# ace19-dev/gvcnn-tf

Hardware: NVIDIA B200
Metric: grouping+fusion shapes/s (12-view, D=2048) (higher is better)
Workload: dtype f32

## Files before the change

gvcnn-tf_b200/build.py:

```python
from __future__ import annotations

import os
import shutil
import subprocess
import sys

HERE = os.path.dirname(os.path.abspath(__file__))
ROOT = os.path.dirname(HERE)
CSRC = os.path.join(HERE, "csrc")
SO = os.path.join(HERE, "libgvcnn_sm100.so")
SOURCES = ["capi.cu", "host_pipeline.cu", "comm.cu", "score.cu", "gap_score.cu", "scheme.cu", "pool_fwd.cu", "pool_fwd_ring.cu", "pool_fwd_direct.cu", "pool_gap_ring.cu", "pool_bwd.cu", "pool_bwd_fast.cu", "paper_mode.cu"]
HEADERS = [os.path.join(CSRC, "common.cuh"), os.path.join(CSRC, "ring_common.cuh"), os.path.join(ROOT, "include", "gvcnn_b200.h")]


def nvcc_path():
    for cand in (shutil.which("nvcc"), "/usr/local/cuda/bin/nvcc"):
        if cand and os.path.exists(cand):
            return cand
    raise RuntimeError("nvcc not found: libgvcnn_sm100.so cannot be built (there is no fallback path)")


def needs_build():
    if not os.path.exists(SO):
        return True
    t = os.path.getmtime(SO)
    deps = [os.path.join(CSRC, s) for s in SOURCES] + HEADERS + [os.path.abspath(__file__)]
    return any(os.path.getmtime(d) > t for d in deps)


def build(force=False, verbose=False, defines=(), out=None):
    if out is None and not force and not needs_build():
        return SO
    import concurrent.futures
    import hashlib
    import tempfile
    target = out or SO
    common = [nvcc_path()]
    if os.path.exists("/usr/bin/g++"):
        common += ["-ccbin", "/usr/bin/g++"]
    common += ["-std=c++17", "-O3", "-lineinfo",
               "-gencode", "arch=compute_100a,code=sm_100a",
               "-fmad=false",
               "-Xcompiler", "-fPIC",
               "-I", os.path.join(ROOT, "include"), "-I", CSRC] + ["-D" + d for d in defines]
    if verbose:
        common.insert(1, "-Xptxas=-v")
    tag = hashlib.sha1((" ".join(defines) + target).encode()).hexdigest()[:10]
    objdir = os.path.join(tempfile.gettempdir(), "gvcnn_build_" + tag)
    os.makedirs(objdir, exist_ok=True)

    def compile_one(src):
        obj = os.path.join(objdir, src.replace(".cu", ".o"))
        res = subprocess.run(common + ["-c", os.path.join(CSRC, src), "-o", obj], capture_output=True, text=True)
        return src, obj, res

    log = []
    objs = []
    with concurrent.futures.ThreadPoolExecutor(max_workers=min(len(SOURCES), os.cpu_count() or 4)) as ex:
        for src, obj, res in ex.map(compile_one, SOURCES):
            log.append(res.stdout + res.stderr)
            if res.returncode != 0:
                sys.stderr.write("".join(log))
                raise RuntimeError("nvcc failed compiling %s" % src)
            objs.append(obj)
    link = common[:1] + (["-ccbin", "/usr/bin/g++"] if os.path.exists("/usr/bin/g++") else []) + \
# ... 16 lines not shown
```

gvcnn-tf_b200/csrc/capi.cu:

```cuda
#include <cstdlib>

#include "comm_dev.cuh"

#ifndef GVCNN_FWD_DIRECT
#define GVCNN_FWD_DIRECT 1
#endif

using namespace gvcnn;

namespace {

size_t elt_size(int dtype) { return dtype == GVCNN_F32 ? 4 : 2; }

int make_view_ptrs(const void *X, int layout, int dtype, int B, int V, int64_t D, ViewPtrs &vp, int64_t &sb,
                   bool &aligned16)
{
    if (!X) return GVCNN_E_BAD_ARG;
    const size_t es = elt_size(dtype);
    char *base = const_cast<char *>(static_cast<const char *>(X));
    switch (layout) {
    case GVCNN_LAYOUT_BVD:
        for (int v = 0; v < V; ++v) vp.p[v] = base + (size_t)v * D * es;
        sb = (int64_t)V * D;
        break;
// ... 291 lines not shown
    if (rc) return rc;
    al = al && is_aligned(dS, 16) && (D * es) % 16 == 0 && (!tie_mask || is_aligned(tie_mask, 8));
    if (weights && (!is_aligned(weights, 4) || weight_stride_b < 0)) return GVCNN_E_BAD_ARG;
    if (al && (variant == 0 || variant == 3 || variant == 4)) {
        rc = launch_pool_fuse_bwd_fast(dS, bins, bin_stride_b, tie_mask, weights, weight_stride_b, gp, sb, status, B, V, D, G, pool, dtype,
                                       static_cast<cudaStream_t>(stream));
        if (rc != -1000) return rc;
    }
    return launch_pool_fuse_bwd(dS, bins, bin_stride_b, tie_mask, weights, weight_stride_b, gp, sb, status, B, V, D, G, pool, dtype, al,
                                static_cast<cudaStream_t>(stream));
}

int gvcnn_grouping_fusion_fwd(const void *R, const float *W, const float *bias, const void *F, float *x,
                              float *scores, int32_t *bins, int32_t *flags, void *S, uint8_t *tie_mask,
                              int32_t *status, int B, int V, int C, int64_t D, int G, int pool, float empty_fill,
                              int r_layout, int f_layout, int dtype, int edge_ulps, int clamp, void *stream)
{
    int rc = check_dims(B, V, D, G, dtype);
    if (rc) return rc == kEmptyBatch ? 0 : rc;
    if (C <= 0 || !W || !bias || !scores || !bins || !S || edge_ulps < 0) return GVCNN_E_BAD_ARG;
    if ((pool & 0xff) != GVCNN_POOL_MAX && (pool & 0xff) != GVCNN_POOL_MEAN) return GVCNN_E_BAD_MODE;
    const size_t es = elt_size(dtype);
    ViewPtrs rp, fp;
    int64_t rsb, fsb;
    bool ral, fal;
    rc = make_view_ptrs(R, r_layout, dtype, B, V, C, rp, rsb, ral);
    if (rc) return rc;
    rc = make_view_ptrs(F, f_layout, dtype, B, V, D, fp, fsb, fal);
    if (rc) return rc;
    (void)es;
    rc = gvcnn_score_bin_fwd(R, W, bias, x, scores, bins, flags, status, B, V, C, G, r_layout, dtype, edge_ulps, clamp,
                             stream);
    if (rc) return rc;
    return pool_fuse_fwd_impl(F, bins, V, nullptr, 0, S, nullptr, tie_mask, status, B, V, D, G, pool, empty_fill,
                               f_layout, dtype, true, stream);
}

int gvcnn_grouping_fusion_batch_fwd(const void *R, const float *W, const float *bias, const void *F, float *x,
                                    float *xsum, float *x_mean, float *scores, int32_t *bins, int32_t *flags, void *S,
                                    uint8_t *tie_mask, int32_t *status, int B, int V, int C, int64_t D, int G,
                                    int multiplier, int pool, float empty_fill, int r_layout, int f_layout, int dtype,
                                    int edge_ulps, int clamp, int64_t global_count, gvcnn_exchange_fn exchange,
                                    void *exchange_user, void *stream)
{
    int rc = check_dims(B, V, D, G, dtype);
    if (rc && rc != kEmptyBatch) return rc;
    const bool empty = rc == kEmptyBatch;
    if (empty && !exchange) return 0;
    if (C <= 0 || !W || !bias || !xsum || !scores || !bins || edge_ulps < 0 || multiplier < 0) return GVCNN_E_BAD_ARG;
    if (!empty && (!x || !S)) return GVCNN_E_BAD_ARG;
    if (global_count < B || global_count <= 0) return GVCNN_E_BAD_ARG;
    if ((pool & 0xff) != GVCNN_POOL_MAX && (pool & 0xff) != GVCNN_POOL_MEAN) return GVCNN_E_BAD_MODE;
    cudaStream_t st = static_cast<cudaStream_t>(stream);
    if (!empty) {
        rc = gvcnn_view_score_fwd(R, W, bias, x, nullptr, B, V, C, r_layout, dtype, stream);
        if (rc) return rc;
    }
    rc = batch_score_tail(empty ? nullptr : x, xsum, x_mean, scores, bins, flags, status, B, V, G, multiplier, edge_ulps,
                          clamp, global_count, exchange, exchange_user, st);
    if (rc || empty) return rc;
    return pool_fuse_fwd_impl(F, bins, 0, nullptr, 0, S, nullptr, tie_mask, status, B, V, D, G, pool, empty_fill,
                               f_layout, dtype, true, stream);
}

size_t gvcnn_pool_fuse_gap_workspace_bytes(int B, int C, int HW, int dtype)
{
    if (B <= 0 || C <= 0 || HW <= 0) return 0;
    return gap_workspace_bytes(B, C, HW, dtype);
}

int gvcnn_pool_fuse_gap_fwd(const void *F, const int32_t *bins, int64_t bin_stride_b, void *S_gap, uint8_t *tie_mask,
                            int32_t *status, void *workspace, size_t workspace_bytes, int B, int V, int HW, int C,
                            int G, int pool, float empty_fill, int f_layout, int dtype, void *stream)
{
    if (HW <= 0 || C <= 0) return GVCNN_E_BAD_ARG;
    const int64_t D = (int64_t)HW * C;
    int rc = check_dims(B, V, D, G, dtype);
    if (rc) return rc == kEmptyBatch ? 0 : rc;
    if (!bins || !S_gap || !workspace || bin_stride_b < 0) return GVCNN_E_BAD_ARG;
    if (pool != GVCNN_POOL_MAX && pool != GVCNN_POOL_MEAN) return GVCNN_E_BAD_MODE;
    ViewPtrs fp;
    int64_t sb;
    bool al;
    rc = make_view_ptrs(F, f_layout, dtype, B, V, D, fp, sb, al);
    if (rc) return rc;
    const size_t need = gap_workspace_bytes(B, C, HW, dtype);
    if (!al || need == 0 || V > 32 || (tie_mask && !is_aligned(tie_mask, 8)) || !is_aligned(workspace, 16))
        return GVCNN_E_UNSUPPORTED;
    if (workspace_bytes < need) return GVCNN_E_WORKSPACE;
    rc = launch_pool_fuse_gap_fwd(fp, sb, bins, bin_stride_b, S_gap, tie_mask, status, static_cast<float *>(workspace),
                                  B, V, HW, C, G, pool, empty_fill, dtype, static_cast<cudaStream_t>(stream));
    return rc == -1000 ? GVCNN_E_UNSUPPORTED : rc;
}

int gvcnn_pool_fuse_gap_bwd(const void *dS_gap, const int32_t *bins, int64_t bin_stride_b, const uint8_t *tie_mask,
                            void *dF, int32_t *status, int B, int V, int HW, int C, int G, int pool, int g_layout,
                            int dtype, void *stream)
{
    if (HW <= 0 || C <= 0) return GVCNN_E_BAD_ARG;
    const int64_t D = (int64_t)HW * C;
    int rc = check_dims(B, V, D, G, dtype);
    if (rc) return rc == kEmptyBatch ? 0 : rc;
    if (!dS_gap || !bins || bin_stride_b < 0) return GVCNN_E_BAD_ARG;
    if (pool != GVCNN_POOL_MAX && pool != GVCNN_POOL_MEAN) return GVCNN_E_BAD_MODE;
    if (pool == GVCNN_POOL_MAX && !tie_mask) return GVCNN_E_BAD_ARG;
    ViewPtrs gp;
// ... 72 lines not shown
```

gvcnn-tf_b200/csrc/common.cuh:

```cuda
#pragma once

#include <cuda_bf16.h>
#include <cuda_runtime.h>
#include <stdint.h>

#include <atomic>
#include <cstdlib>

#include "gvcnn_b200.h"

namespace gvcnn {

struct ViewPtrs {
    char *p[GVCNN_MAX_VIEWS];
};

struct Plan {
    int32_t rawbin[GVCNN_MAX_VIEWS];
    int32_t gbin[GVCNN_MAX_VIEWS];
    float gw[GVCNN_MAX_VIEWS];
    float sumw;
    uint16_t glen[GVCNN_MAX_VIEWS];
    uint8_t order[GVCNN_MAX_VIEWS];
};
// ... 418 lines not shown
    const float lo = fmaxf(ax - dx, 0.0f), hi = ax + dx;
    float s_lo = __fdiv_rn(lo, __fadd_rn(1.0f, lo)), s_hi = __fdiv_rn(hi, __fadd_rn(1.0f, hi));
    const uint32_t bl = __float_as_uint(s_lo), bh = __float_as_uint(s_hi);
    s_lo = __uint_as_float(bl > (uint32_t)edge_ulps ? bl - edge_ulps : 0u);
    s_hi = __uint_as_float(bh + edge_ulps);
    const float fg = (float)(mult > 0 ? mult : G);
    return ((int)__fmul_rn(s_lo, fg) != (int)__fmul_rn(s_hi, fg)) ? GVCNN_FLAG_ORDER_EDGE : 0;
}

__device__ __forceinline__ void publish(int flags, int32_t *flag_out, int32_t *status)
{
    if (flag_out) *flag_out = flags;
    if (status && flags) {
        if (flags & GVCNN_FLAG_BIN_RANGE) atomicAdd(status + GVCNN_STATUS_BIN_RANGE, 1);
        if (flags & GVCNN_FLAG_NAN) atomicAdd(status + GVCNN_STATUS_NAN, 1);
        if (flags & GVCNN_FLAG_NEAR_EDGE) atomicAdd(status + GVCNN_STATUS_NEAR_EDGE, 1);
    }
}

int launch_view_score(const ViewPtrs &rp, int64_t r_sb, const float *W, const float *bias, float *x, float *xabs,
                      float *scores, int32_t *bins, int32_t *flags, int32_t *status, int B, int V, int C,
                      int G, int dtype, bool aligned16, bool fuse_bin, int edge_ulps, int clamp,
                      cudaStream_t st);
int launch_gap_score(const ViewPtrs &mp, int64_t m_sb, const float *W, const float *bias, float *R_out, float *x,
                     float *scores, int32_t *bins, int32_t *flags, int32_t *status, int B, int V, int HW, int C, int G,
                     int dtype, bool fuse_bin, int edge_ulps, int clamp, cudaStream_t st);
int launch_batch_sum_x(const float *x, float *xsum, int B, int V, cudaStream_t st);
int launch_score_bin(const float *x, float denom, float *x_mean, float *scores, int32_t *bins, int32_t *flags,
                     int32_t *status, int64_t n, int G, int multiplier, int edge_ulps, int clamp, bool x_is_score,
                     const float *xabs, int bound_terms, cudaStream_t st);
int launch_bins_to_scheme(const int32_t *bins, int32_t *scheme, int rows, int V, int G, cudaStream_t st);
int launch_scheme_to_bins(const int32_t *scheme, int32_t *bins, int32_t *status, int rows, int V, int G,
                          cudaStream_t st);
int launch_group_weight(const int32_t *bins, float *weights, int rows, int V, int G, cudaStream_t st);
int launch_pool_fuse_fwd(const ViewPtrs &fp, int64_t f_sb, const int32_t *bins, int64_t bin_sb, void *S,
                         void *Pout, uint8_t *mask, const float *weights, int64_t w_sb, int32_t *status, int B, int V, int64_t D, int G, int pool,
                         float fill, int dtype, bool aligned16, int variant, cudaStream_t st);
int launch_group_weight_from_scores(const float *scores, const int32_t *bins, float *weights, int rows, int V, int G,
                                    cudaStream_t st);
int launch_group_weight_grad(const ViewPtrs &fp, int64_t f_sb, const void *dS, const void *S, const int32_t *bins,
                             int64_t bin_sb, const float *weights, int64_t w_sb, float *dweights, int B, int V,
                             int64_t D, int G, int pool, int dtype, bool aligned16, cudaStream_t st);
int launch_score_weight_bwd(const float *dweights, const int32_t *bins, const float *x, float *dx, int rows, int V,
                            int G, cudaStream_t st);
int launch_view_score_bwd(const ViewPtrs &rp, int64_t r_sb, const float *dx, const float *W, float *dW, float *dbias,
                          const ViewPtrs &drp, int64_t dr_sb, int want_dr, float *workspace, int NS, int B, int V,
                          int C, int dtype, bool aligned16, cudaStream_t st);
int launch_pool_fuse_fwd_ring(const ViewPtrs &fp, int64_t f_sb, const int32_t *bins, int64_t bin_sb,
                              const float *weights, int64_t w_sb, void *S, uint8_t *mask, int32_t *status, int B, int V, int64_t D, int G, int pool,
                              float fill, int dtype, cudaStream_t st);
int launch_pool_fuse_fwd_direct(const ViewPtrs &fp, int64_t f_sb, const int32_t *bins, int64_t bin_sb, void *S,
                                uint8_t *mask, int32_t *status, int B, int V, int64_t D, int G, int pool, float fill,
                                int dtype, bool forced, bool f_ready, cudaStream_t st);
size_t gap_workspace_bytes(int B, int C, int HW, int dtype);
int launch_pool_fuse_gap_fwd(const ViewPtrs &fp, int64_t f_sb, const int32_t *bins, int64_t bin_sb, void *out,
                             uint8_t *mask, int32_t *status, float *partial, int B, int V, int HW, int C, int G,
                             int pool, float fill, int dtype, cudaStream_t st);
int launch_pool_fuse_gap_bwd(const void *dOut, const int32_t *bins, int64_t bin_sb, const uint8_t *mask,
                             const ViewPtrs &gp, int64_t g_sb, int32_t *status, int B, int V, int HW, int C, int G,
                             int pool, int dtype, cudaStream_t st);
int launch_pool_fuse_bwd_fast(const void *dS, const int32_t *bins, int64_t bin_sb, const uint8_t *mask,
                              const float *weights, int64_t w_sb, const ViewPtrs &gp, int64_t g_sb, int32_t *status, int B, int V, int64_t D, int G,
                              int pool, int dtype, cudaStream_t st);
int launch_pool_fuse_bwd(const void *dS, const int32_t *bins, int64_t bin_sb, const uint8_t *mask,
                         const float *weights, int64_t w_sb,
                         const ViewPtrs &gp, int64_t g_sb, int32_t *status, int B, int V, int64_t D, int G,
                         int pool, int dtype, bool aligned16, cudaStream_t st);

}
```

gvcnn-tf_b200/csrc/score.cu:

```cuda
#include "comm_dev.cuh"

namespace gvcnn {

constexpr int kScoreWarps = 8;
constexpr int kScoreUnroll = 8;

template <typename T, bool VEC, bool FUSE_BIN, bool BOUND>
__global__ void __launch_bounds__(kScoreWarps * 32)
view_score_kernel(const ViewPtrs rp, const int64_t r_sb, const float *__restrict__ W,
                  const float *__restrict__ bias, float *__restrict__ x_out, float *__restrict__ xabs_out,
                  float *__restrict__ scores,
                  int32_t *__restrict__ bins, int32_t *__restrict__ flag_out, int32_t *status, const int B,
                  const int V, const int C, const int G, const int edge_ulps, const int clamp)
{
    constexpr int E = VEC ? Elem<T>::kVec : 1;
    const int lane = threadIdx.x & 31;
    const int64_t row = (int64_t)blockIdx.x * kScoreWarps + (threadIdx.x >> 5);
    pdl_wait();
    pdl_launch_dependents();
    if (row >= (int64_t)B * V) return;
    const int b = (int)(row / V);
    const int v = (int)(row - (int64_t)b * V);
    const T *__restrict__ r = reinterpret_cast<const T *>(rp.p[v]) + (int64_t)b * r_sb;
    const float *__restrict__ w = W + (int64_t)v * C;

    float acc = 0.0f, aabs = 0.0f;
    if constexpr (VEC) {
        for (int base0 = lane * E; base0 < C; base0 += 32 * E * kScoreUnroll) {
            uint4 raw[kScoreUnroll];
#pragma unroll
            for (int u = 0; u < kScoreUnroll; ++u) {
                const int base = base0 + u * 32 * E;
                if (base < C) raw[u] = ldg_stream_16(r + base);
            }
#pragma unroll
            for (int u = 0; u < kScoreUnroll; ++u) {
                const int base = base0 + u * 32 * E;
                if (base < C) {
                    float f[E];
                    Elem<T>::unpack(raw[u], f);
#pragma unroll
                    for (int j = 0; j < E; j += 4) {
                        const float4 wv = __ldg(reinterpret_cast<const float4 *>(w + base + j));
                        acc = fmaf(f[j + 0], wv.x, acc);
                        acc = fmaf(f[j + 1], wv.y, acc);
                        acc = fmaf(f[j + 2], wv.z, acc);
                        acc = fmaf(f[j + 3], wv.w, acc);
                        if constexpr (BOUND) {
                            aabs = fmaf(fabsf(f[j + 0]), fabsf(wv.x), aabs);
                            aabs = fmaf(fabsf(f[j + 1]), fabsf(wv.y), aabs);
                            aabs = fmaf(fabsf(f[j + 2]), fabsf(wv.z), aabs);
                            aabs = fmaf(fabsf(f[j + 3]), fabsf(wv.w), aabs);
                        }
                    }
                }
            }
        }
    } else {
        for (int c = lane; c < C; c += 32) {
            const float rv = Elem<T>::to_float(r[c]), wv = __ldg(w + c);
            acc = fmaf(rv, wv, acc);
            if constexpr (BOUND) aabs = fmaf(fabsf(rv), fabsf(wv), aabs);
        }
    }
#pragma unroll
    for (int off = 16; off >= 1; off >>= 1) acc = __fadd_rn(acc, __shfl_xor_sync(0xffffffffu, acc, off));
    if constexpr (BOUND) {
#pragma unroll
        for (int off = 16; off >= 1; off >>= 1) aabs = __fadd_rn(aabs, __shfl_xor_sync(0xffffffffu, aabs, off));
    }

    if (lane == 0) {
        const float bv = __ldg(bias + v);
        const float x = __fadd_rn(acc, bv);
        const float A = BOUND ? __fadd_rn(aabs, fabsf(bv)) : 0.0f;
        if (x_out) x_out[row] = x;
        if constexpr (BOUND && !FUSE_BIN) xabs_out[row] = A;
        if constexpr (FUSE_BIN) {
            float s;
            int bin;
            int flags = score_and_bin(x, 1.0f, G, edge_ulps, clamp, s, bin);
            if constexpr (BOUND) flags |= order_edge_flag(x, A, C + 2, G, 0, edge_ulps);
            scores[row] = s;
            bins[row] = bin;
            publish(flags, flag_out ? flag_out + row : nullptr, status);
        }
    }
}

constexpr int kFastRows = 4;

__device__ __forceinline__ float transpose_reduce4(const float (&acc)[4], const int lane)
{
    const bool hi = (lane & 16) != 0;
    float k0 = hi ? acc[2] : acc[0], k1 = hi ? acc[3] : acc[1];
    const float s0 = hi ? acc[0] : acc[2], s1 = hi ? acc[1] : acc[3];
    k0 = __fadd_rn(k0, __shfl_xor_sync(0xffffffffu, s0, 16));
    k1 = __fadd_rn(k1, __shfl_xor_sync(0xffffffffu, s1, 16));
    const bool h8 = (lane & 8) != 0;
    float k = h8 ? k1 : k0;
    const float sd = h8 ? k0 : k1;
    k = __fadd_rn(k, __shfl_xor_sync(0xffffffffu, sd, 8));
#pragma unroll
    for (int off = 4; off >= 1; off >>= 1) k = __fadd_rn(k, __shfl_xor_sync(0xffffffffu, k, off));
    return k;
}

template <typename T, int NB, bool BOUND>
__global__ void __launch_bounds__(kScoreWarps * 32)
view_score_fast_kernel(const ViewPtrs rp, const int64_t r_sb, const float *__restrict__ W,
                       const float *__restrict__ bias, float *__restrict__ x_out, float *__restrict__ xabs_out,
                       float *__restrict__ scores,
                       int32_t *__restrict__ bins, int32_t *__restrict__ flag_out, int32_t *status, const int B,
                       const int V, const int G, const int edge_ulps, const int clamp, const int64_t items,
                       const int rpw)
{
    constexpr int E = Elem<T>::kVec;
    constexpr int C = NB * 32 * E;
    const int lane = threadIdx.x & 31;
    const int64_t item = (int64_t)blockIdx.x * kScoreWarps + (threadIdx.x >> 5);
    pdl_wait();
    pdl_launch_dependents();
    if (item >= items) return;
    const int v = (int)(item % V);
    const int b_first = (int)(item / V) * rpw;
    const int b_end = min(b_first + rpw, B);
    const T *__restrict__ r0 = reinterpret_cast<const T *>(rp.p[v]) + lane * E;
    const float *__restrict__ w = W + (int64_t)v * C + lane * E;
    const float bv = __ldg(bias + v);
#ifndef GVCNN_SCORE_PD_MAX
#define GVCNN_SCORE_PD_MAX kFastRows
#endif
    constexpr int PD = (16 / NB) < GVCNN_SCORE_PD_MAX ? (16 / NB < 2 ? 2 : 16 / NB) : GVCNN_SCORE_PD_MAX;
    uint4 buf[PD][NB];
#pragma unroll
    for (int j = 0; j < PD; ++j) {
        if (b_first + j < b_end) {
            const T *rn = r0 + (int64_t)(b_first + j) * r_sb;
#pragma unroll
            for (int u = 0; u < NB; ++u) buf[j][u] = ldg_stream_16(rn + u * 32 * E);
        } else {
#pragma unroll
            for (int u = 0; u < NB; ++u) buf[j][u] = make_uint4(0u, 0u, 0u, 0u);
        }
    }
    for (int b0 = b_first; b0 < b_end; b0 += kFastRows) {
        float acc[kFastRows], aabs[kFastRows];
#pragma unroll
        for (int j = 0; j < kFastRows; ++j) {
            float a = 0.0f, aa = 0.0f;
#pragma unroll
            for (int u = 0; u < NB; ++u) {
                float f[E];
                Elem<T>::unpack(buf[j % PD][u], f);
#pragma unroll
                for (int q = 0; q < E; q += 4) {
                    const float4 wv = __ldg(reinterpret_cast<const float4 *>(w + u * 32 * E + q));
                    a = fmaf(f[q + 0], wv.x, a);
                    a = fmaf(f[q + 1], wv.y, a);
                    a = fmaf(f[q + 2], wv.z, a);
                    a = fmaf(f[q + 3], wv.w, a);
                    if constexpr (BOUND) {
                        aa = fmaf(fabsf(f[q + 0]), fabsf(wv.x), aa);
                        aa = fmaf(fabsf(f[q + 1]), fabsf(wv.y), aa);
                        aa = fmaf(fabsf(f[q + 2]), fabsf(wv.z), aa);
                        aa = fmaf(fabsf(f[q + 3]), fabsf(wv.w), aa);
                    }
                }
            }
            acc[j] = a;
            aabs[j] = aa;
            const int bn = b0 + j + PD;
            if (bn < b_end) {
                const T *rn = r0 + (int64_t)bn * r_sb;
#pragma unroll
                for (int u = 0; u < NB; ++u) buf[j % PD][u] = ldg_stream_16(rn + u * 32 * E);
            }
        }
        const float k = transpose_reduce4(acc, lane);
        const float ka = BOUND ? transpose_reduce4(aabs, lane) : 0.0f;

        const int b = b0 + (lane >> 3);
        if ((lane & 7) == 0 && b < b_end) {
            const int64_t row = (int64_t)b * V + v;
            const float x = __fadd_rn(k, bv);
            const float A = BOUND ? __fadd_rn(ka, fabsf(bv)) : 0.0f;
            if (x_out) x_out[row] = x;
            if constexpr (BOUND) {
                if (xabs_out) xabs_out[row] = A;
            }
            if (scores) {
                float s;
                int bin;
                int flags = score_and_bin(x, 1.0f, G, edge_ulps, clamp, s, bin);
                if constexpr (BOUND) flags |= order_edge_flag(x, A, C + 2, G, 0, edge_ulps);
                scores[row] = s;
                bins[row] = bin;
                publish(flags, flag_out ? flag_out + row : nullptr, status);
            }
        }
    }
}

__global__ void __launch_bounds__(256) batch_sum_x_kernel(const float *__restrict__ x,
                                                          float *__restrict__ xsum, const int B, const int V)
{
    __shared__ float warp_sum[8];
    const int v = blockIdx.x;
    pdl_wait();
    pdl_launch_dependents();
    float acc = 0.0f;
    for (int b = threadIdx.x; b < B; b += 256) acc = __fadd_rn(acc, x[(int64_t)b * V + v]);
#pragma unroll
    for (int off = 16; off >= 1; off >>= 1) acc = __fadd_rn(acc, __shfl_xor_sync(0xffffffffu, acc, off));
    if ((threadIdx.x & 31) == 0) warp_sum[threadIdx.x >> 5] = acc;
    __syncthreads();
    if (threadIdx.x == 0) {
        float t = warp_sum[0];
        for (int i = 1; i < 8; ++i) t = __fadd_rn(t, warp_sum[i]);
        xsum[v] = t;
    }
}

__global__ void __launch_bounds__(256) score_bin_kernel(const float *__restrict__ x, const float denom,
                                                        float *__restrict__ x_mean, float *__restrict__ scores,
                                                        int32_t *__restrict__ bins,
                                                        int32_t *__restrict__ flag_out, int32_t *status,
                                                        const int64_t n, const int G, const int mult,
                                                        const int edge_ulps, const int clamp,
                                                        const bool x_is_score, const float *__restrict__ xabs,
                                                        const int bound_terms)
{
    const int64_t i = (int64_t)blockIdx.x * 256 + threadIdx.x;
    pdl_wait();
    pdl_launch_dependents();
    if (i >= n) return;
    float s;
    int bin;
    int flags = score_and_bin(x[i], denom, G, edge_ulps, clamp, s, bin, x_is_score, mult);
    if (xabs && !x_is_score)
        flags |= order_edge_flag(__fdiv_rn(x[i], denom), __fdiv_rn(xabs[i], denom), bound_terms, G, mult, edge_ulps);
    if (x_mean) x_mean[i] = __fdiv_rn(x[i], denom);
    if (scores) scores[i] = s;
    bins[i] = bin;
    publish(flags, flag_out ? flag_out + i : nullptr, status);
}

template <bool COMM>
__global__ void __launch_bounds__(256)
batch_mean_bin_fused_kernel(const float *__restrict__ x, float *__restrict__ xsum, float *__restrict__ x_mean,
                            float *__restrict__ scores, int32_t *__restrict__ bins, int32_t *__restrict__ flag_out,
                            int32_t *status, const int B, const int V, const int G, const int mult, const int edge_ulps,
                            const int clamp, const float denom, const CommPeers peers, const int rank, const int world)
{
    __shared__ float warp_sum[8];
    __shared__ float parts[kCommMaxWorld];
    const int v = blockIdx.x;
    pdl_wait();
    pdl_launch_dependents();
    float acc = 0.0f;
    for (int b = threadIdx.x; b < B; b += 256) acc = __fadd_rn(acc, x[(int64_t)b * V + v]);
#pragma unroll
    for (int off = 16; off >= 1; off >>= 1) acc = __fadd_rn(acc, __shfl_xor_sync(0xffffffffu, acc, off));
    if ((threadIdx.x & 31) == 0) warp_sum[threadIdx.x >> 5] = acc;
    __syncthreads();
    float sum = 0.0f;
    if (threadIdx.x < 32) {
        sum = warp_sum[0];
        for (int i = 1; i < 8; ++i) sum = __fadd_rn(sum, warp_sum[i]);
        if constexpr (COMM) {
            CommBuf *mine = peers.buf[rank];
            const int lane = threadIdx.x;
            const uint32_t seq = mine->seqv[v] + 1u;
            const int phase = (int)(seq & 1u);
            __syncwarp();
            if (lane == 0) mine->seqv[v] = seq;
            if (lane < world) ll_store1(&peers.buf[(rank + 1 + lane) % world]->llv[phase][rank][v], sum, seq);
            float val = 0.0f;
            if (lane < world && !ll_wait1(&mine->llv[phase][lane][v], seq, val, comm_timer_ns())) atomicExch(&mine->error, 1u);
            sum = __shfl_sync(0xffffffffu, val, 0);
            for (int r = 1; r < world; ++r) sum = __fadd_rn(sum, __shfl_sync(0xffffffffu, val, r));
        }
    }
    if (threadIdx.x == 0) {
        xsum[v] = sum;
        float s;
        int bin;
        const int flags = score_and_bin(sum, denom, G, edge_ulps, clamp, s, bin, false, mult);
        if (x_mean) x_mean[v] = __fdiv_rn(sum, denom);
        if (scores) scores[v] = s;
        bins[v] = bin;
        publish(flags, flag_out ? flag_out + v : nullptr, status);
    }
}

int launch_batch_mean_bin_fused(const float *x, float *xsum, float *x_mean, float *scores, int32_t *bins, int32_t *flags,
                                int32_t *status, int B, int V, int G, int multiplier, int edge_ulps, int clamp,
                                float denom, const CommPeers *peers, int rank, int world, cudaStream_t st)
{
    if (V > GVCNN_MAX_VIEWS) return -1000;
    cudaError_t err;
    if (peers && world > 1) {
        err = launch_pdl(batch_mean_bin_fused_kernel<true>, dim3(V), dim3(256), 0, st, x, xsum, x_mean, scores, bins,
                         flags, status, B, V, G, multiplier, edge_ulps, clamp, denom, *peers, rank, world);
    } else {
        CommPeers none = {};
        err = launch_pdl(batch_mean_bin_fused_kernel<false>, dim3(V), dim3(256), 0, st, x, xsum, x_mean, scores, bins,
                         flags, status, B, V, G, multiplier, edge_ulps, clamp, denom, none, 0, 1);
    }
    if (err != cudaSuccess) return (int)err;
    return (int)cudaGetLastError();
}

static int score_sm_count()
{
    static int cached = 0;
    if (cached == 0) {
        int dev = 0, n = 0;
        if (cudaGetDevice(&dev) != cudaSuccess ||
            cudaDeviceGetAttribute(&n, cudaDevAttrMultiProcessorCount, dev) != cudaSuccess || n <= 0) {
            cudaGetLastError();
            return 148;
        }
        cached = n;
    }
    return cached;
}

template <typename T>
static int launch_view_score_t(const ViewPtrs &rp, int64_t r_sb, const float *W, const float *bias, float *x,
                               float *xabs, float *scores, int32_t *bins, int32_t *flags, int32_t *status, int B, int V,
                               int C, int G, bool vec, bool fuse_bin, int edge_ulps, int clamp,
                               cudaStream_t st)
{
    const int64_t rows = (int64_t)B * V;
    const bool bound = fuse_bin ? (flags != nullptr) : (xabs != nullptr);
    cudaError_t err = cudaSuccess;
    if (vec && (C == 8 * 32 * Elem<T>::kVec || C == 4 * 32 * Elem<T>::kVec)) {
        static const int env_rpw = env_int_once("GVCNN_SCORE_RPW", 0);
        const dim3 fblock(kScoreWarps * 32);
#define GVCNN_LAUNCH_FAST(NB_, BOUND_)                                                                       \
    do {                                                                                                     \
        const int64_t warp_slots = (int64_t)score_sm_count() *                                               \
            resident_ctas<view_score_fast_kernel<T, NB_, BOUND_>>(kScoreWarps * 32) * kScoreWarps;           \
        int rpw = (int)(kFastRows * ((rows + kFastRows * warp_slots - 1) / (kFastRows * warp_slots)));       \
        if (env_rpw >= kFastRows && env_rpw % kFastRows == 0) rpw = env_rpw;                                 \
// ... 69 lines not shown
```

Before: 37.16 million.

## Fuse view scoring, batch binning and pooling into one cooperative persistent kernel

Adds a single cooperative kernel for the non-exchange, default-variant batch forward path. It computes view scores with bulk async row loads, grid-syncs to reduce the batch mean and assign bins, then runs a TMA-fed ring pooling stage. The first pooling stages are prefetched before the grid syncs so the F loads overlap the scoring and binning. This replaces three separate launches and their inter-kernel gaps, at the cost of two grid-wide barriers, a fixed V=12 and C=1024 specialisation, and a fallback path when those preconditions are not met.

```diff
diff --git a/gvcnn-tf_b200/build.py b/gvcnn-tf_b200/build.py
--- a/gvcnn-tf_b200/build.py
+++ b/gvcnn-tf_b200/build.py
@@ -9,8 +9,8 @@
 ROOT = os.path.dirname(HERE)
 CSRC = os.path.join(HERE, "csrc")
 SO = os.path.join(HERE, "libgvcnn_sm100.so")
-SOURCES = ["capi.cu", "host_pipeline.cu", "comm.cu", "score.cu", "gap_score.cu", "scheme.cu", "pool_fwd.cu", "pool_fwd_ring.cu", "pool_fwd_direct.cu", "pool_gap_ring.cu", "pool_bwd.cu", "pool_bwd_fast.cu", "paper_mode.cu"]
-HEADERS = [os.path.join(CSRC, "common.cuh"), os.path.join(CSRC, "ring_common.cuh"), os.path.join(ROOT, "include", "gvcnn_b200.h")]
+SOURCES = ["capi.cu", "host_pipeline.cu", "comm.cu", "score.cu", "gap_score.cu", "scheme.cu", "pool_fwd.cu", "pool_fwd_ring.cu", "pool_fwd_direct.cu", "fwd_batch_fused.cu", "pool_gap_ring.cu", "pool_bwd.cu", "pool_bwd_fast.cu", "paper_mode.cu"]
+HEADERS = [os.path.join(CSRC, "common.cuh"), os.path.join(CSRC, "ring_common.cuh"), os.path.join(CSRC, "score_common.cuh"), os.path.join(ROOT, "include", "gvcnn_b200.h")]
 
 
 def nvcc_path():
diff --git a/gvcnn-tf_b200/csrc/capi.cu b/gvcnn-tf_b200/csrc/capi.cu
--- a/gvcnn-tf_b200/csrc/capi.cu
+++ b/gvcnn-tf_b200/csrc/capi.cu
@@ -367,6 +367,20 @@
     if (global_count < B || global_count <= 0) return GVCNN_E_BAD_ARG;
     if ((pool & 0xff) != GVCNN_POOL_MAX && (pool & 0xff) != GVCNN_POOL_MEAN) return GVCNN_E_BAD_MODE;
     cudaStream_t st = static_cast<cudaStream_t>(stream);
+    if (!empty && !exchange && GVCNN_POOL_VARIANT_OF(pool) == 0) {
+        ViewPtrs rp, fp;
+        int64_t rsb, fsb;
+        bool ral, fal;
+        if (make_view_ptrs(R, r_layout, dtype, B, V, C, rp, rsb, ral) == 0 &&
+            make_view_ptrs(F, f_layout, dtype, B, V, D, fp, fsb, fal) == 0 && ral && fal && is_aligned(W, 16) &&
+            is_aligned(bias, 4) && is_aligned(x, 4) && is_aligned(bins, 4) && is_aligned(S, 16) &&
+            (!tie_mask || is_aligned(tie_mask, 8))) {
+            rc = launch_fwd_batch_fused(rp, rsb, W, bias, x, xsum, x_mean, scores, bins, flags, status, fp, fsb, S,
+                                        tie_mask, B, V, C, D, G, multiplier, pool, empty_fill, edge_ulps, clamp,
+                                        (float)global_count, dtype, st);
+            if (rc != -1000) return rc;
+        }
+    }
     if (!empty) {
         rc = gvcnn_view_score_fwd(R, W, bias, x, nullptr, B, V, C, r_layout, dtype, stream);
         if (rc) return rc;
diff --git a/gvcnn-tf_b200/csrc/common.cuh b/gvcnn-tf_b200/csrc/common.cuh
--- a/gvcnn-tf_b200/csrc/common.cuh
+++ b/gvcnn-tf_b200/csrc/common.cuh
@@ -494,6 +494,11 @@
 int launch_pool_fuse_fwd_direct(const ViewPtrs &fp, int64_t f_sb, const int32_t *bins, int64_t bin_sb, void *S,
                                 uint8_t *mask, int32_t *status, int B, int V, int64_t D, int G, int pool, float fill,
                                 int dtype, bool forced, bool f_ready, cudaStream_t st);
+int launch_fwd_batch_fused(const ViewPtrs &rp, int64_t r_sb, const float *W, const float *bias, float *x, float *xsum,
+                           float *x_mean, float *scores, int32_t *bins, int32_t *flags, int32_t *status,
+                           const ViewPtrs &fp, int64_t f_sb, void *S, uint8_t *mask, int B, int V, int C, int64_t D,
+                           int G, int multiplier, int pool, float fill, int edge_ulps, int clamp, float denom, int dtype,
+                           cudaStream_t st);
 size_t gap_workspace_bytes(int B, int C, int HW, int dtype);
 int launch_pool_fuse_gap_fwd(const ViewPtrs &fp, int64_t f_sb, const int32_t *bins, int64_t bin_sb, void *out,
                              uint8_t *mask, int32_t *status, float *partial, int B, int V, int HW, int C, int G,
diff --git a/gvcnn-tf_b200/csrc/fwd_batch_fused.cu b/gvcnn-tf_b200/csrc/fwd_batch_fused.cu
--- /dev/null
+++ b/gvcnn-tf_b200/csrc/fwd_batch_fused.cu
@@ -0,0 +1,382 @@
+#include <cooperative_groups.h>
+
+#include "ring_common.cuh"
+#include "score_common.cuh"
+
+namespace gvcnn {
+
+#ifdef GVCNN_FUSED_TRACE
+__device__ unsigned long long g_fused_trace[8 * 1024];
+#define GVCNN_FUSED_MARK(slot_)                                                             \
+    do {                                                                                    \
+        unsigned long long t_;                                                              \
+        asm volatile("mov.u64 %0, %%globaltimer;" : "=l"(t_));                              \
+        if (blockIdx.x < 1024) g_fused_trace[8 * blockIdx.x + (slot_)] = t_;                \
+    } while (0)
+#else
+#define GVCNN_FUSED_MARK(slot_) do { } while (0)
+#endif
+
+constexpr int kFusedMaxRowBufs = 8;
+
+struct FusedBatchArgs {
+    const float *W, *bias;
+    float *x, *xsum, *x_mean, *scores;
+    int32_t *bins, *flags, *status;
+    void *S;
+    uint8_t *mask;
+    int64_t r_sb, f_sb, D, items;
+    int B, G, mult, edge_ulps, clamp, rpw, row_bufs, stages, tiles_per_shape, num_tiles;
+    float denom, fill;
+};
+
+template <typename T, int POOL, bool MASK, int V, int NB, int NCONS, int MINB>
+__global__ void __launch_bounds__(NCONS + kRingProducerThreads, MINB)
+fwd_batch_fused_kernel(const ViewPtrs rp, const ViewPtrs fp, const FusedBatchArgs a)
+{
+    constexpr int E = Elem<T>::kVec;
+    constexpr int C = NB * 32 * E;
+    constexpr int kConsWarps = NCONS / 32;
+    constexpr uint32_t kRBytes = (uint32_t)C * sizeof(T);
+    constexpr int TD = NCONS * E;
+    constexpr uint32_t kRowStride = (uint32_t)NCONS * 16u;
+    constexpr uint32_t kStageBytes = kRowStride * (uint32_t)V;
+    constexpr int kMaxStages = 8;
+    extern __shared__ __align__(128) unsigned char smem_raw[];
+    __shared__ RingPlan plan;
+    __shared__ int32_t sorted_bin[32];
+    __shared__ uint8_t rank_of[32];
+    __shared__ float warp_sum[8];
+    __shared__ __align__(8) uint64_t full_bar[kMaxStages];
+    __shared__ __align__(8) uint64_t empty_bar[kMaxStages];
+    __shared__ __align__(8) uint64_t r_bar[kConsWarps * kFusedMaxRowBufs];
+
+    const int warp = threadIdx.x >> 5, lane = threadIdx.x & 31;
+    const bool producer = warp == kConsWarps;
+    if (threadIdx.x == 0) {
+        GVCNN_FUSED_MARK(0);
+        for (int s = 0; s < a.stages; ++s) {
+            mbar_init(&full_bar[s], 1);
+            mbar_init(&empty_bar[s], (uint32_t)kConsWarps);
+        }
+        for (int i = 0; i < kConsWarps * a.row_bufs; ++i) mbar_init(&r_bar[i], 1);
+        mbar_fence_init();
+    }
+    __syncthreads();
+    pdl_wait();
+    pdl_launch_dependents();
+    const uint64_t policy = l2_policy_evict_first();
+
+    if (!producer) {
+        unsigned char *rbuf = smem_raw + (size_t)warp * a.row_bufs * kRBytes;
+        uint64_t *rbar = r_bar + warp * a.row_bufs;
+        uint32_t rph = 0;
+        const int64_t nwarps = (int64_t)gridDim.x * kConsWarps;
+        for (int64_t item = (int64_t)warp * gridDim.x + blockIdx.x; item < a.items; item += nwarps) {
+            const int v = (int)(item % V);
+            const int b_first = (int)(item / V) * a.rpw;
+            const int b_end = min(b_first + a.rpw, a.B);
+            const char *r0 = rp.p[v];
+            auto issue = [&](const int slot, const int b) {
+                mbar_expect_tx(&rbar[slot], kRBytes);
+                bulk_g2s_hint(rbuf + (size_t)slot * kRBytes, r0 + (int64_t)b * a.r_sb * (int64_t)sizeof(T), kRBytes,
+                              &rbar[slot], policy);
+            };
+            if (lane == 0)
+                for (int j = 0; j < a.row_bufs && b_first + j < b_end; ++j) issue(j, b_first + j);
+            float4 wr[NB * E / 4];
+            const float *w = a.W + (int64_t)v * C + lane * E;
+#pragma unroll
+            for (int u = 0; u < NB; ++u)
+#pragma unroll
+                for (int q = 0; q < E; q += 4) wr[(u * E + q) / 4] = __ldg(reinterpret_cast<const float4 *>(w + u * 32 * E + q));
+            const float bv = __ldg(a.bias + v);
+            for (int b0 = b_first; b0 < b_end; b0 += kFastRows) {
+                float acc[kFastRows];
+#pragma unroll
+                for (int j = 0; j < kFastRows; ++j) {
+                    float pa = 0.0f, pabs = 0.0f;
+                    const int bj = b0 + j;
+                    if (bj < b_end) {
+                        const int slot = (bj - b_first) % a.row_bufs;
+                        mbar_wait(&rbar[slot], (rph >> slot) & 1u);
+                        rph ^= 1u << slot;
+                        uint4 raw[NB];
+#pragma unroll
+                        for (int u = 0; u < NB; ++u)
+                            raw[u] = *reinterpret_cast<const uint4 *>(rbuf + (size_t)slot * kRBytes + u * 512 + lane * 16);
+                        __syncwarp();
+                        if (lane == 0 && bj + a.row_bufs < b_end) issue(slot, bj + a.row_bufs);
+                        score_row_partial<T, NB, false>(raw, [&](int u, int q) { return wr[(u * E + q) / 4]; }, pa, pabs);
+                    }
+                    acc[j] = pa;
+                }
+                const float k = transpose_reduce4(acc, lane);
+                const int b = b0 + (lane >> 3);
+                if ((lane & 7) == 0 && b < b_end) a.x[(int64_t)b * V + v] = __fadd_rn(k, bv);
+            }
+        }
+    }
+    if (threadIdx.x == 0) GVCNN_FUSED_MARK(1);
+#ifdef GVCNN_FUSED_R_ONLY
+    return;
+#endif
+
+    asm volatile("fence.proxy.async.shared::cta;" ::: "memory");
+    __syncthreads();
+    const int step_b = (int)gridDim.x / a.tiles_per_shape;
+    const int step_t = (int)gridDim.x - step_b * a.tiles_per_shape;
+    const int b_start = (int)blockIdx.x / a.tiles_per_shape;
+    const int tile_start = (int)blockIdx.x - b_start * a.tiles_per_shape;
+    if (producer && lane < V) {
+        int b = b_start, tile = tile_start;
+        for (int it = 0, t = blockIdx.x; it < a.stages && t < a.num_tiles; ++it, t += gridDim.x) {
+            const int64_t d0 = (int64_t)tile * TD;
+            const uint32_t row_bytes = (uint32_t)min((int64_t)TD, a.D - d0) * sizeof(T);
+            if (lane == 0) mbar_expect_tx(&full_bar[it], row_bytes * (uint32_t)V);
+            __syncwarp((1u << V) - 1u);
+            bulk_g2s_hint(smem_raw + (size_t)it * kStageBytes + (size_t)lane * kRowStride,
+                          fp.p[lane] + ((int64_t)b * a.f_sb + d0) * (int64_t)sizeof(T), row_bytes, &full_bar[it], policy);
+            b += step_b;
+            tile += step_t;
+            if (tile >= a.tiles_per_shape) { tile -= a.tiles_per_shape; ++b; }
+        }
+    }
+    cooperative_groups::grid_group grid = cooperative_groups::this_grid();
+    grid.sync();
+    if (threadIdx.x == 0) GVCNN_FUSED_MARK(2);
+    if ((int)blockIdx.x < V && threadIdx.x < 256) {
+        const int v = blockIdx.x;
+        batch_xsum_partial<true>(a.x, a.B, V, v, warp_sum);
+        asm volatile("bar.sync 1, 256;" ::: "memory");
+        if (threadIdx.x == 0)
+            batch_bin_publish(batch_xsum_total(warp_sum), v, a.xsum, a.x_mean, a.scores, a.bins, a.flags, a.status,
+                              a.G, a.mult, a.edge_ulps, a.clamp, a.denom);
+    }
+    grid.sync();
+    if (threadIdx.x == 0) GVCNN_FUSED_MARK(3);
+
+    int nbad = 0, k = 0;
+    if (producer) {
+        int bin = 0x7fffffff;
+        bool bad = false;
+        if (lane < V) {
+            bin = __ldcg(a.bins + lane);
+            if (bin < 0 || bin >= a.G) {
+                bad = true;
+                bin = bin < 0 ? 0 : a.G - 1;
+            }
+        }
+        nbad = __popc(__ballot_sync(0xffffffffu, bad));
+        int below = 0, same_before = 0;
+#pragma unroll
+        for (int u = 0; u < V; ++u) {
+            const int bu = __shfl_sync(0xffffffffu, bin, u);
+            below += (bu < bin);
+            same_before += (bu == bin) & (u < lane);
+        }
+        k = below + same_before;
+        const bool first = lane < V && same_before == 0;
+        const uint32_t fm = __reduce_or_sync(0xffffffffu, first ? (1u << k) : 0u);
+        if (lane < V) sorted_bin[k] = bin;
+        __syncwarp();
+        const int prev = (lane < V && k > 0) ? sorted_bin[k - 1] : -1;
+        const int last_bin = sorted_bin[V - 1];
+        if (lane < V) {
+            plan.skip[k] = (uint8_t)(first ? bin - prev - 1 : 0);
+            rank_of[lane] = (uint8_t)k;
+        }
+        if (lane == 0) {
+            plan.first_mask = fm;
+            plan.tail_skip = (uint32_t)(a.G - 1 - last_bin);
+        }
+    }
+    __syncthreads();
+
+    int b = b_start, tile = tile_start, s = 0;
+    uint32_t ph = 0;
+    if (producer) {
+        for (int it = 0, t = blockIdx.x; t < a.num_tiles; ++it, t += gridDim.x) {
+            if (lane == 0 && nbad && a.status && tile == 0) atomicAdd(a.status + GVCNN_STATUS_BIN_RANGE, nbad);
+            if (it >= a.stages) {
+                const int64_t d0 = (int64_t)tile * TD;
+                const uint32_t row_bytes = (uint32_t)min((int64_t)TD, a.D - d0) * sizeof(T);
+                if (lane == 0) mbar_wait(&empty_bar[s], ph ^ 1u);
+                __syncwarp();
+                if (lane == 0) mbar_expect_tx(&full_bar[s], row_bytes * (uint32_t)V);
+                __syncwarp();
+                if (lane < V)
+                    bulk_g2s_hint(smem_raw + (size_t)s * kStageBytes + (size_t)k * kRowStride,
+                                  fp.p[lane] + ((int64_t)b * a.f_sb + d0) * (int64_t)sizeof(T), row_bytes, &full_bar[s],
+                                  policy);
+            }
+            b += step_b;
+            tile += step_t;
+            if (tile >= a.tiles_per_shape) { tile -= a.tiles_per_shape; ++b; }
+            if (++s == a.stages) { s = 0; ph ^= 1u; }
+        }
+    } else {
+        T *S = static_cast<T *>(a.S);
+        const int e0 = threadIdx.x * E;
+        const float sumw = (float)(a.G + V);
+        const float rcp_sumw = __frcp_rn(sumw);
+        for (int it = 0, t = blockIdx.x; t < a.num_tiles; ++it, t += gridDim.x) {
+            const int64_t d0 = (int64_t)tile * TD;
+            const bool active = (int64_t)e0 < a.D - d0;
+            const int64_t out_off = (int64_t)b * a.D + d0 + e0;
+            unsigned char *col = smem_raw + (size_t)s * kStageBytes + (size_t)threadIdx.x * 16;
+            mbar_wait(&full_bar[s], ph);
+            if (it < a.stages && active) {
+                uint4 raw[V];
+#pragma unroll
+                for (int v = 0; v < V; ++v) raw[v] = *reinterpret_cast<const uint4 *>(col + v * kRowStride);
+#pragma unroll
+                for (int v = 0; v < V; ++v) *reinterpret_cast<uint4 *>(col + (uint32_t)rank_of[v] * kRowStride) = raw[v];
+            }
+            float acc[E];
+            ring_consume_tile<T, POOL, MASK, V, kRowStride>(col, plan, a.fill, active, a.mask, a.B, a.D, out_off, acc);
+            __syncwarp();
+            if (lane == 0) mbar_arrive(&empty_bar[s]);
+            if (threadIdx.x == 0 && it == 0) GVCNN_FUSED_MARK(4);
+            if (active) {
+                div_vec_by_rcp(acc, sumw, rcp_sumw);
+                stg_stream_16(S + out_off, Elem<T>::pack(acc));
+            }
+            b += step_b;
+            tile += step_t;
+            if (tile >= a.tiles_per_shape) { tile -= a.tiles_per_shape; ++b; }
+            if (++s == a.stages) { s = 0; ph ^= 1u; }
+        }
+    }
+    if (threadIdx.x == 0) GVCNN_FUSED_MARK(5);
+}
+
+namespace {
+
+struct FusedDevice {
+    int sms = 0;
+    int coop = 0;
+};
+int fused_device(FusedDevice &out)
+{
+    static FusedDevice cache[64];
+    static std::atomic<int> known[64];
+    int dev = 0;
+    cudaError_t e = cudaGetDevice(&dev);
+    if (e != cudaSuccess) return (int)e;
+    if (dev < 0 || dev >= 64) return -1000;
+    if (!known[dev].load(std::memory_order_acquire)) {
+        FusedDevice d;
+        if (cudaDeviceGetAttribute(&d.sms, cudaDevAttrMultiProcessorCount, dev) != cudaSuccess ||
+            cudaDeviceGetAttribute(&d.coop, cudaDevAttrCooperativeLaunch, dev) != cudaSuccess) {
+            cudaGetLastError();
+            return -1000;
+        }
+        cache[dev] = d;
+        known[dev].store(1, std::memory_order_release);
+    }
+    out = cache[dev];
+    return 0;
+}
+
+template <typename T, int V, int NB>
+int launch_fused_v(const ViewPtrs &rp, const ViewPtrs &fp, FusedBatchArgs a, int pool, bool want_mask, int sms,
+                   cudaStream_t st)
+{
+    constexpr int NCONS = 256, MINB = 2;
+    constexpr int E = Elem<T>::kVec;
+    constexpr size_t stage_bytes = (size_t)V * NCONS * 16;
+    constexpr size_t r_bytes = (size_t)NB * 32 * 16;
+    int stages = (int)(((226 * 1024) / MINB - 3 * 1024) / stage_bytes);
+    if (stages > 8) stages = 8;
+    if (stages < 2) return -1000;
+    const size_t smem = stage_bytes * stages;
+    int row_bufs = (int)(smem / (r_bytes * (NCONS / 32)));
+    if (row_bufs > kFusedMaxRowBufs) row_bufs = kFusedMaxRowBufs;
+    if (row_bufs < 2) return -1000;
+    const int64_t td = (int64_t)NCONS * E;
+    const int64_t tps = (a.D + td - 1) / td;
+    const int64_t tiles = (int64_t)a.B * tps;
+    if (tiles > 0x7fffffffLL) return GVCNN_E_BAD_ARG;
+    a.stages = stages;
+    a.row_bufs = row_bufs;
+    a.tiles_per_shape = (int)tps;
+    a.num_tiles = (int)tiles;
+    cudaError_t err = cudaSuccess;
+#define GVCNN_LAUNCH_FUSED(POOL_, MASK_)                                                                            \
+    do {                                                                                                            \
+        constexpr auto kern = fwd_batch_fused_kernel<T, POOL_, MASK_, V, NB, NCONS, MINB>;                          \
+        err = ensure_dyn_smem<kern>((int)smem);                                                                     \
+        if (err != cudaSuccess) break;                                                                              \
+        const int per_sm = resident_ctas<kern>(NCONS + kRingProducerThreads, smem);                                 \
+        const int grid = sms * per_sm;                                                                              \
+         \
+        const int64_t rows = (int64_t)a.B * V, warp_slots = (int64_t)grid * (NCONS / 32);                           \
+        a.rpw = (int)(kFastRows * ((rows + kFastRows * warp_slots - 1) / (kFastRows * warp_slots)));                \
+        a.items = (int64_t)V * ((a.B + a.rpw - 1) / a.rpw);                                                         \
+        cudaLaunchConfig_t cfg = {};                                                                                \
+        cfg.gridDim = dim3(grid);                                                                                   \
+        cfg.blockDim = dim3(NCONS + kRingProducerThreads);                                                          \
+        cfg.dynamicSmemBytes = smem;                                                                                \
+        cfg.stream = st;                                                                                            \
+        cudaLaunchAttribute attr[2];                                                                                \
+        attr[0].id = cudaLaunchAttributeCooperative;                                                                \
+        attr[0].val.cooperative = 1;                                                                                \
+        attr[1].id = cudaLaunchAttributeProgrammaticStreamSerialization;                                            \
+        attr[1].val.programmaticStreamSerializationAllowed = 1;                                                     \
+        cfg.attrs = attr;                                                                                           \
+        cfg.numAttrs = 2;                                                                                           \
+        err = cudaLaunchKernelEx(&cfg, kern, rp, fp, a);                                                            \
+    } while (0)
+    if (pool == GVCNN_POOL_MAX) {
+        if (want_mask) GVCNN_LAUNCH_FUSED(GVCNN_POOL_MAX, true); else GVCNN_LAUNCH_FUSED(GVCNN_POOL_MAX, false);
+    } else {
+        GVCNN_LAUNCH_FUSED(GVCNN_POOL_MEAN, false);
+    }
+#undef GVCNN_LAUNCH_FUSED
+    if (err != cudaSuccess) return (int)err;
+    return (int)cudaGetLastError();
+}
+
+}
+
+int launch_fwd_batch_fused(const ViewPtrs &rp, int64_t r_sb, const float *W, const float *bias, float *x, float *xsum,
+                           float *x_mean, float *scores, int32_t *bins, int32_t *flags, int32_t *status,
+                           const ViewPtrs &fp, int64_t f_sb, void *S, uint8_t *mask, int B, int V, int C, int64_t D,
+                           int G, int multiplier, int pool, float fill, int edge_ulps, int clamp, float denom, int dtype,
+                           cudaStream_t st)
+{
+    if (B <= 0 || V != 12 || G > 255) return -1000;
+    const int E = dtype == GVCNN_F32 ? 4 : 8;
+    if (D % E || D < 256 * E) return -1000;
+    FusedDevice dev;
+    if (fused_device(dev) != 0 || !dev.coop) return -1000;
+    FusedBatchArgs a = {};
+    a.W = W;
+    a.bias = bias;
+    a.x = x;
+    a.xsum = xsum;
+    a.x_mean = x_mean;
+    a.scores = scores;
+    a.bins = bins;
+    a.flags = flags;
+    a.status = status;
+    a.S = S;
+    a.mask = pool == GVCNN_POOL_MAX ? mask : nullptr;
+    a.r_sb = r_sb;
+    a.f_sb = f_sb;
+    a.D = D;
+    a.B = B;
+    a.G = G;
+    a.mult = multiplier;
+    a.edge_ulps = edge_ulps;
+    a.clamp = clamp;
+    a.denom = denom;
+    a.fill = fill;
+    const bool want_mask = a.mask != nullptr;
+    if (C != 1024) return -1000;
+    if (dtype == GVCNN_F32) return launch_fused_v<float, 12, 8>(rp, fp, a, pool, want_mask, dev.sms, st);
+    return launch_fused_v<__nv_bfloat16, 12, 4>(rp, fp, a, pool, want_mask, dev.sms, st);
+}
+
+}
diff --git a/gvcnn-tf_b200/csrc/score.cu b/gvcnn-tf_b200/csrc/score.cu
--- a/gvcnn-tf_b200/csrc/score.cu
+++ b/gvcnn-tf_b200/csrc/score.cu
@@ -1,4 +1,5 @@
 #include "comm_dev.cuh"
+#include "score_common.cuh"
 
 namespace gvcnn {
 
@@ -88,24 +89,6 @@
     }
 }
 
-constexpr int kFastRows = 4;
-
-__device__ __forceinline__ float transpose_reduce4(const float (&acc)[4], const int lane)
-{
-    const bool hi = (lane & 16) != 0;
-    float k0 = hi ? acc[2] : acc[0], k1 = hi ? acc[3] : acc[1];
-    const float s0 = hi ? acc[0] : acc[2], s1 = hi ? acc[1] : acc[3];
-    k0 = __fadd_rn(k0, __shfl_xor_sync(0xffffffffu, s0, 16));
-    k1 = __fadd_rn(k1, __shfl_xor_sync(0xffffffffu, s1, 16));
-    const bool h8 = (lane & 8) != 0;
-    float k = h8 ? k1 : k0;
-    const float sd = h8 ? k0 : k1;
-    k = __fadd_rn(k, __shfl_xor_sync(0xffffffffu, sd, 8));
-#pragma unroll
-    for (int off = 4; off >= 1; off >>= 1) k = __fadd_rn(k, __shfl_xor_sync(0xffffffffu, k, off));
-    return k;
-}
-
 template <typename T, int NB, bool BOUND>
 __global__ void __launch_bounds__(kScoreWarps * 32)
 view_score_fast_kernel(const ViewPtrs rp, const int64_t r_sb, const float *__restrict__ W,
@@ -148,26 +131,10 @@
         float acc[kFastRows], aabs[kFastRows];
 #pragma unroll
         for (int j = 0; j < kFastRows; ++j) {
-            float a = 0.0f, aa = 0.0f;
-#pragma unroll
-            for (int u = 0; u < NB; ++u) {
-                float f[E];
-                Elem<T>::unpack(buf[j % PD][u], f);
-#pragma unroll
-                for (int q = 0; q < E; q += 4) {
-                    const float4 wv = __ldg(reinterpret_cast<const float4 *>(w + u * 32 * E + q));
-                    a = fmaf(f[q + 0], wv.x, a);
-                    a = fmaf(f[q + 1], wv.y, a);
-                    a = fmaf(f[q + 2], wv.z, a);
-                    a = fmaf(f[q + 3], wv.w, a);
-                    if constexpr (BOUND) {
-                        aa = fmaf(fabsf(f[q + 0]), fabsf(wv.x), aa);
-                        aa = fmaf(fabsf(f[q + 1]), fabsf(wv.y), aa);
-                        aa = fmaf(fabsf(f[q + 2]), fabsf(wv.z), aa);
-                        aa = fmaf(fabsf(f[q + 3]), fabsf(wv.w), aa);
-                    }
-                }
-            }
+            float a, aa;
+            score_row_partial<T, NB, BOUND>(
+                buf[j % PD], [&](int u, int q) { return __ldg(reinterpret_cast<const float4 *>(w + u * 32 * E + q)); },
+                a, aa);
             acc[j] = a;
             aabs[j] = aa;
             const int bn = b0 + j + PD;
@@ -258,16 +225,11 @@
     const int v = blockIdx.x;
     pdl_wait();
     pdl_launch_dependents();
-    float acc = 0.0f;
-    for (int b = threadIdx.x; b < B; b += 256) acc = __fadd_rn(acc, x[(int64_t)b * V + v]);
-#pragma unroll
-    for (int off = 16; off >= 1; off >>= 1) acc = __fadd_rn(acc, __shfl_xor_sync(0xffffffffu, acc, off));
-    if ((threadIdx.x & 31) == 0) warp_sum[threadIdx.x >> 5] = acc;
+    batch_xsum_partial<false>(x, B, V, v, warp_sum);
     __syncthreads();
     float sum = 0.0f;
     if (threadIdx.x < 32) {
-        sum = warp_sum[0];
-        for (int i = 1; i < 8; ++i) sum = __fadd_rn(sum, warp_sum[i]);
+        sum = batch_xsum_total(warp_sum);
         if constexpr (COMM) {
             CommBuf *mine = peers.buf[rank];
             const int lane = threadIdx.x;
@@ -282,16 +244,8 @@
             for (int r = 1; r < world; ++r) sum = __fadd_rn(sum, __shfl_sync(0xffffffffu, val, r));
         }
     }
-    if (threadIdx.x == 0) {
-        xsum[v] = sum;
-        float s;
-        int bin;
-        const int flags = score_and_bin(sum, denom, G, edge_ulps, clamp, s, bin, false, mult);
-        if (x_mean) x_mean[v] = __fdiv_rn(sum, denom);
-        if (scores) scores[v] = s;
-        bins[v] = bin;
-        publish(flags, flag_out ? flag_out + v : nullptr, status);
-    }
+    if (threadIdx.x == 0)
+        batch_bin_publish(sum, v, xsum, x_mean, scores, bins, flag_out, status, G, mult, edge_ulps, clamp, denom);
 }
 
 int launch_batch_mean_bin_fused(const float *x, float *xsum, float *x_mean, float *scores, int32_t *bins, int32_t *flags,
diff --git a/gvcnn-tf_b200/csrc/score_common.cuh b/gvcnn-tf_b200/csrc/score_common.cuh
--- /dev/null
+++ b/gvcnn-tf_b200/csrc/score_common.cuh
@@ -0,0 +1,97 @@
+#pragma once
+
+#include "common.cuh"
+
+namespace gvcnn {
+
+constexpr int kFastRows = 4;
+
+__device__ __forceinline__ float transpose_reduce4(const float (&acc)[4], const int lane)
+{
+    const bool hi = (lane & 16) != 0;
+    float k0 = hi ? acc[2] : acc[0], k1 = hi ? acc[3] : acc[1];
+    const float s0 = hi ? acc[0] : acc[2], s1 = hi ? acc[1] : acc[3];
+    k0 = __fadd_rn(k0, __shfl_xor_sync(0xffffffffu, s0, 16));
+    k1 = __fadd_rn(k1, __shfl_xor_sync(0xffffffffu, s1, 16));
+    const bool h8 = (lane & 8) != 0;
+    float k = h8 ? k1 : k0;
+    const float sd = h8 ? k0 : k1;
+    k = __fadd_rn(k, __shfl_xor_sync(0xffffffffu, sd, 8));
+#pragma unroll
+    for (int off = 4; off >= 1; off >>= 1) k = __fadd_rn(k, __shfl_xor_sync(0xffffffffu, k, off));
+    return k;
+}
+
+template <typename T, int NB, bool BOUND, typename WQ>
+__device__ __forceinline__ void score_row_partial(const uint4 (&raw)[NB], WQ wq, float &a, float &aa)
+{
+    constexpr int E = Elem<T>::kVec;
+    a = 0.0f;
+    aa = 0.0f;
+#pragma unroll
+    for (int u = 0; u < NB; ++u) {
+        float f[E];
+        Elem<T>::unpack(raw[u], f);
+#pragma unroll
+        for (int q = 0; q < E; q += 4) {
+            const float4 wv = wq(u, q);
+            a = fmaf(f[q + 0], wv.x, a);
+            a = fmaf(f[q + 1], wv.y, a);
+            a = fmaf(f[q + 2], wv.z, a);
+            a = fmaf(f[q + 3], wv.w, a);
+            if constexpr (BOUND) {
+                aa = fmaf(fabsf(f[q + 0]), fabsf(wv.x), aa);
+                aa = fmaf(fabsf(f[q + 1]), fabsf(wv.y), aa);
+                aa = fmaf(fabsf(f[q + 2]), fabsf(wv.z), aa);
+                aa = fmaf(fabsf(f[q + 3]), fabsf(wv.w), aa);
+            }
+        }
+    }
+}
+
+template <bool COHERENT>
+__device__ __forceinline__ void batch_xsum_partial(const float *x, const int B, const int V, const int v,
+                                                   float *warp_sum)
+{
+    constexpr int kAhead = 16;
+    float acc = 0.0f;
+    for (int b0 = threadIdx.x; b0 < B; b0 += 256 * kAhead) {
+        float t[kAhead];
+#pragma unroll
+        for (int j = 0; j < kAhead; ++j) {
+            const int b = b0 + j * 256;
+            t[j] = 0.0f;
+            if (b < B) t[j] = COHERENT ? __ldcg(x + (int64_t)b * V + v) : __ldg(x + (int64_t)b * V + v);
+        }
+#pragma unroll
+        for (int j = 0; j < kAhead; ++j)
+            if (b0 + j * 256 < B) acc = __fadd_rn(acc, t[j]);
+    }
+#pragma unroll
+    for (int off = 16; off >= 1; off >>= 1) acc = __fadd_rn(acc, __shfl_xor_sync(0xffffffffu, acc, off));
+    if ((threadIdx.x & 31) == 0) warp_sum[threadIdx.x >> 5] = acc;
+}
+
+__device__ __forceinline__ float batch_xsum_total(const float *warp_sum)
+{
+    float sum = warp_sum[0];
+    for (int i = 1; i < 8; ++i) sum = __fadd_rn(sum, warp_sum[i]);
+    return sum;
+}
+
+__device__ __forceinline__ void batch_bin_publish(const float sum, const int v, float *xsum, float *x_mean,
+                                                  float *scores, int32_t *bins, int32_t *flag_out, int32_t *status,
+                                                  const int G, const int mult, const int edge_ulps, const int clamp,
+                                                  const float denom)
+{
+    xsum[v] = sum;
+    float s;
+    int bin;
+    const int flags = score_and_bin(sum, denom, G, edge_ulps, clamp, s, bin, false, mult);
+    if (x_mean) x_mean[v] = __fdiv_rn(sum, denom);
+    if (scores) scores[v] = s;
+    bins[v] = bin;
+    publish(flags, flag_out ? flag_out + v : nullptr, status);
+}
+
+}
```

Measured after the change: 37.93 million (median of 6 runs). 2.1% higher.
